# Go2Heart/StreamFormer

Hardware: AMD Instinct MI355X
Metric: frames/s (16x224^2 clips) (higher is better)
Workload: dtype bf16; 1 GPU; SigLIP-base StreamFormer encoder forward, 8 clips x 16 x 224^2 per GPU, random-init de-trivialised weights, causal temporal attention; global_batch_clips=8, frames_per_clip=16, parallelism=dp1, steps_in_flight=1

## Files before the change

include/streamformer_hip.h:

```cpp
#ifndef STREAMFORMER_HIP_H
#define STREAMFORMER_HIP_H

#include <stddef.h>
#include <stdint.h>

#ifdef __cplusplus
extern "C" {
#endif

typedef struct sf_encoder sf_encoder;
typedef struct sf_cache sf_cache;
typedef void* sf_stream;

typedef enum {
  SF_OK = 0,
  SF_ERR_INVALID = -1,
  SF_ERR_STATE = -2,
  SF_ERR_HIP = -3,
  SF_ERR_WORKSPACE = -4,
  SF_ERR_UNKNOWN_KEY = -5,
  SF_ERR_CAPACITY = -6
} sf_status;

typedef enum { SF_F32 = 0, SF_BF16 = 1, SF_F16 = 2, SF_F64 = 3, SF_U8 = 4 } sf_dtype;
// ... 395 lines not shown
int sf_op_crit_losses_backward(const float* const* pred_masks, int L, int B, int Q, int H, int W, const float* const* tgt_masks,
                               const int32_t* tgt_G, const int32_t* tgt_H, const int32_t* tgt_W, const int32_t* pairs_dev, int N,
                               const float* coords_dev, const float* sums_dev, int K, float num_masks, const float* upstream_dev,
                               float* grad_pred_masks_dev, sf_stream stream);
size_t sf_op_crit_class_loss_workspace_bytes(int L, int B, int Q);
int sf_op_crit_class_loss(const float* const* pred_logits, int L, int B, int Q, int C1, const int32_t* pairs_dev, int N,
                          const int64_t* const* tgt_labels, const int32_t* tgt_G, const float* weight_dev, float* losses_dev,
                          int losses_stride, float* grad_dev, int32_t* target_classes_out_dev, void* workspace, size_t workspace_bytes,
                          sf_stream stream);

int sf_op_clp_tracks(const float* embeds_dev, int R, int C, const int32_t* track_rows_dev, int T, int F, float* sg_dev, float* stats_dev,
                     sf_stream stream);
int sf_op_clp_items(const float* embeds_dev, int R, int C, const float* sg_dev, int T, int F, const int32_t* items_dev, int I,
                    const int32_t* neg_dev, int NE, int max_neg, float* losses_dev, float* item_out_dev, sf_stream stream);
size_t sf_op_clp_backward_workspace_bytes(int I, int T, int F, int C);
int sf_op_clp_backward(const float* embeds_dev, int R, int C, const float* sg_dev, const float* stats_dev, const int32_t* track_rows_dev,
                       const int32_t* track_items_dev, int T, int F, const int32_t* items_dev, int I, const int32_t* neg_dev, int NE,
                       int max_neg, const int32_t* row_start_dev, const int32_t* row_items_dev, const float* item_out_dev,
                       const float* upstream_dev, float* grad_embeds_dev, void* workspace, size_t workspace_bytes, sf_stream stream);

int sf_bench_gemm(sf_encoder* enc, int M, int which, int iters, void* workspace_dev,
                  size_t workspace_bytes, sf_stream stream, float* mean_ms_out, double* flops_out);

int sf_bench_attention(sf_encoder* enc, int B, int T, int which, int iters, void* workspace_dev,
                       size_t workspace_bytes, sf_stream stream, float* mean_ms_out, double* bytes_out,
                       double* flops_out);

void sf_reload_switches(void);
const char* sf_switch_info(int index, int what);

int sf_bench_launch_floor(int device, int launches, int iters, sf_stream stream, float* us_per_launch_out);

#ifdef __cplusplus
}
#endif
#endif
```

streamformer_amd/_native.py:

```python
from __future__ import annotations

import ctypes as C
import inspect
import os
import weakref

import torch

_HERE = os.path.dirname(os.path.abspath(__file__))
LIB_PATH = os.path.join(_HERE, "libstreamformer_hip.so")
if os.environ.get("SF_LIB"):
    LIB_PATH = os.path.join(_HERE, "libstreamformer_hip_%s.so" % os.environ["SF_LIB"])

SF_OK = 0
SF_ERR_INVALID, SF_ERR_STATE, SF_ERR_HIP, SF_ERR_WORKSPACE, SF_ERR_UNKNOWN_KEY, SF_ERR_CAPACITY = -1, -2, -3, -4, -5, -6
SF_F32, SF_BF16, SF_F16, SF_F64, SF_U8 = 0, 1, 2, 3, 4
SF_COMPUTE_BF16, SF_COMPUTE_BF16X3 = 0, 1


class SfConfig(C.Structure):
    _fields_ = [(n, C.c_int32) for n in (
        "image_size", "patch_size", "num_channels", "num_frames", "hidden_size", "num_hidden_layers",
        "num_attention_heads", "intermediate_size", "hidden_act", "qkv_bias", "enable_causal_temporal",
        "add_lora_spatial")] + [("layer_norm_eps", C.c_float)]
# ... 215 lines not shown
    "sf_op_seg_semantic": (_I, [_P, _P, _I, _I, _I, _I, _I, _I, _I, _I, _I, _I, _P, _P]),
    "sf_op_seg_panoptic_argmax": (_I, [_P, _P, _P, _I, _I, _F, _I, _I, _I, _I, _I, _I, _I, _I, _P, _P, _P]),
    "sf_op_seg_panoptic_relabel": (_I, [_P, _P, _I, C.c_longlong, _P, _P]),
    "sf_op_crit_costs_workspace_bytes": (_SZ, [_I, _I, _I, _I, _I]),
    "sf_op_crit_costs": (_I, [C.POINTER(_P), C.POINTER(_P), _I, _I, _I, _I, _I, _I, C.POINTER(_P), C.POINTER(_P), C.POINTER(C.c_int32),
                              C.POINTER(C.c_int32), C.POINTER(C.c_int32), _P, _I, _I, _F, _F, _F, _P, _P, _SZ, _P]),
    "sf_op_crit_losses_capacity": (_I, []),
    "sf_op_crit_losses_workspace_bytes": (_SZ, [_I]),
    "sf_op_crit_losses": (_I, [C.POINTER(_P), _I, _I, _I, _I, _I, C.POINTER(_P), C.POINTER(C.c_int32), C.POINTER(C.c_int32),
                               C.POINTER(C.c_int32), _P, C.POINTER(C.c_int32), _I, _P, _P, _I, _I, _I, _F, _P, _I, _P, _P, _P, _P, _SZ, _P]),
    "sf_op_crit_losses_backward": (_I, [C.POINTER(_P), _I, _I, _I, _I, _I, C.POINTER(_P), C.POINTER(C.c_int32), C.POINTER(C.c_int32),
                                        C.POINTER(C.c_int32), _P, _I, _P, _P, _I, _F, _P, _P, _P]),
    "sf_op_crit_class_loss_workspace_bytes": (_SZ, [_I, _I, _I]),
    "sf_op_crit_class_loss": (_I, [C.POINTER(_P), _I, _I, _I, _I, _P, _I, C.POINTER(_P), C.POINTER(C.c_int32), _P, _P, _I, _P, _P, _P, _SZ,
                                   _P]),
    "sf_op_clp_tracks": (_I, [_P, _I, _I, _P, _I, _I, _P, _P, _P]),
    "sf_op_clp_items": (_I, [_P, _I, _I, _P, _I, _I, _P, _I, _P, _I, _I, _P, _P, _P]),
    "sf_op_clp_backward_workspace_bytes": (_SZ, [_I, _I, _I, _I]),
    "sf_op_clp_backward": (_I, [_P, _I, _I, _P, _P, _P, _P, _I, _I, _P, _I, _P, _I, _I, _P, _P, _P, _P, _P, _P, _SZ, _P]),
    "sf_reload_switches": (None, []),
    "sf_switch_info": (C.c_char_p, [_I, _I]),
    "sf_bench_launch_floor": (_I, [_I, _I, _I, _P, C.POINTER(_F)]),
    "sf_bench_gemm": (_I, [_P, _I, _I, _I, _P, _SZ, _P, C.POINTER(_F), C.POINTER(C.c_double)]),
    "sf_bench_attention": (_I, [_P, _I, _I, _I, _I, _P, _SZ, _P, C.POINTER(_F), C.POINTER(C.c_double),
                                C.POINTER(C.c_double)]),
}


def _load() -> C.CDLL:
    if not os.path.exists(LIB_PATH):
        raise ImportError(
            f"{LIB_PATH} is missing: build it with `python streamformer_amd/build.py` "
            "(hipcc --offload-arch=gfx950).  There is no non-HIP fallback.")
    lib = C.CDLL(LIB_PATH, mode=C.RTLD_GLOBAL)
    for name, (res, args) in SIGNATURES.items():
        try:
            fn = getattr(lib, name)
        except AttributeError as e:
            raise ImportError(f"{LIB_PATH} does not export {name} (stale build? run "
                              "`python streamformer_amd/build.py`)") from e
        fn.restype = res
        fn.argtypes = args
    return lib


lib = _load()
# ... 165 lines not shown
```

streamformer_amd/csrc/sf_bench.hip:

```cpp
#include "sf_encoder.h"

#include <cstring>

template <typename Launch>
static hipError_t sf_time_launches(hipStream_t s, int iters, Launch&& launch, float* mean_ms) {
  hipEvent_t e0 = nullptr, e1 = nullptr;
  hipError_t err = hipEventCreate(&e0);
  if (err == hipSuccess) err = hipEventCreate(&e1);
  if (err == hipSuccess) err = launch();
  if (err == hipSuccess) err = hipEventRecord(e0, s);
  for (int i = 0; i < iters && err == hipSuccess; ++i) err = launch();
  if (err == hipSuccess) err = hipEventRecord(e1, s);
  if (err == hipSuccess) err = hipEventSynchronize(e1);
  float ms = 0.f;
  if (err == hipSuccess) err = hipEventElapsedTime(&ms, e0, e1);
  if (e0) (void)hipEventDestroy(e0);
  if (e1) (void)hipEventDestroy(e1);
  if (err == hipSuccess) *mean_ms = ms / iters;
  return err;
}

extern "C" int sf_bench_gemm(sf_encoder* e, int M, int which, int iters, void* workspace, size_t workspace_bytes,
                             sf_stream stream, float* mean_ms_out, double* flops_out) {
  if (!e || !e->finalized || e->layers.empty()) return sf_set_err(SF_ERR_STATE, "encoder not finalized");
  if (iters <= 0 || M <= 0 || !workspace || !mean_ms_out) return sf_set_err(SF_ERR_INVALID, "bad argument");
  const DevLayer& l = e->layers[0];
  const bool plain = which == 4 || which == 5;
  if (plain) which = which == 4 ? 3 : 1;
  const DevLinear* lin = which == 0 ? &l.up : which == 1 ? &l.down : which == 2 ? &l.s_qkv : &l.s_out;
  const bool acc = e->compute == SF_COMPUTE_BF16X3;
  const int epi = plain ? (acc ? SF_EPI_F32 : SF_EPI_BF16) : which == 0 ? SF_EPI_ACT_BF16 : which == 2 ? (acc ? SF_EPI_F32 : SF_EPI_BF16) : SF_EPI_RESID_F32;
  const bool pm = epi == SF_EPI_RESID_F32 && resid_planes_at(e, M);
  SfCarver c(workspace, acc || pm, true);
  const SfPlanes ap = c.planes((size_t)M * lin->K);
  SfPlanes op = c.planes((size_t)M * lin->N);
  float* of = c.take<float>((size_t)M * lin->N);
  if (c.off > workspace_bytes) return sf_set_err(SF_ERR_WORKSPACE, "workspace %zu < required %zu", workspace_bytes, c.off);
  hipStream_t s = (hipStream_t)stream;
  if (acc && epi == SF_EPI_RESID_F32) op.hi = nullptr;
  float* st = pm ? c.take<float>((size_t)M * 8) : nullptr;
  if (c.off > workspace_bytes) return sf_set_err(SF_ERR_WORKSPACE, "workspace %zu < required %zu", workspace_bytes, c.off);
  if (st) HIP_TRY(hipMemsetAsync(st, 0, (size_t)M * 8 * sizeof(float), (hipStream_t)stream));
  SfGemmArgs g = linear_args(e, *lin, ap.hi, ap.lo, M, epi, acc);
  g.alpha = 0.f; g.out_hi = op.hi; g.out_lo = op.lo;
  if (pm) { g.resid_hi = op.hi; g.resid_lo = op.lo; g.ln_stats_out = st; }
  else { g.out_f32 = of; g.resid = of; }
  HIP_TRY(sf_time_launches(s, iters, [&]() { return sf_launch_gemm(g, acc, s); }, mean_ms_out));
  if (flops_out) *flops_out = 2.0 * M * (double)lin->N * (double)lin->K;
  return SF_OK;
}

extern "C" int sf_bench_attention(sf_encoder* e, int B, int T, int which, int iters, void* workspace,
                                  size_t workspace_bytes, sf_stream stream, float* mean_ms_out, double* bytes_out,
                                  double* flops_out) {
  if (!e || !e->finalized) return sf_set_err(SF_ERR_STATE, "encoder not finalized");
  if (iters <= 0 || B <= 0 || T <= 0 || !workspace || !mean_ms_out) return sf_set_err(SF_ERR_INVALID, "bad argument");
  const bool acc = e->compute == SF_COMPUTE_BF16X3;
  const int D = e->D, N = e->N, heads = e->cfg.num_attention_heads;
  const size_t M = (size_t)B * T * N, esz = acc ? 4 : 2;
  SfCarver c(workspace);
  char* qkv = c.take<char>(M * 3 * D * esz);
  bf16_t* ch = c.take<bf16_t>(M * D);
  bf16_t* cl = c.take<bf16_t>(M * D);
  if (c.off > workspace_bytes) return sf_set_err(SF_ERR_WORKSPACE, "workspace %zu < required %zu", workspace_bytes, c.off);
  hipStream_t s = (hipStream_t)stream;
  HIP_TRY(hipMemsetAsync(qkv, 0x3c, M * 3 * D * esz, s));
  SfAttnArgs a;
  memset(&a, 0, sizeof(a));
  a.q = qkv; a.k = qkv + (size_t)D * esz; a.v = qkv + (size_t)2 * D * esz;
  a.in_is_f32 = acc; a.row_pitch_q = 3 * D; a.row_pitch_kv = 3 * D; a.heads = heads; a.scale = 0.125f;
  a.ctx_hi = ch; a.ctx_lo = cl; a.D = D; a.N = N;
  if (which == 0 && acc && sf_spatial_planes_ok(N, false)) {
// ... 66 lines not shown
```

streamformer_amd/csrc/sf_common.h:

```cpp
#pragma once
#include <hip/hip_runtime.h>
#include <stdint.h>

typedef unsigned short bf16_t;

typedef __attribute__((ext_vector_type(8))) short bf16x8_t;
typedef __attribute__((ext_vector_type(4))) float f32x4_t;
typedef __attribute__((ext_vector_type(4))) unsigned int u32x4_t;
typedef __attribute__((ext_vector_type(2))) unsigned int u32x2_t;

#define SF_DEVICE __device__ __forceinline__

#ifdef SF_LAB
#define SF_LAB_SWITCH(name) (getenv(name) ? atoi(getenv(name)) : 0)
#else
#define SF_LAB_SWITCH(name) 0
#endif

SF_DEVICE int sf_swz64(int row) {
#ifdef SF_SWZ64_LEGACY
  return (row >> 2) & 3;
#else
  return (0 - (row >> 2)) & 3;
#endif
// ... 200 lines not shown
  if (p.grp_rows <= 0) return (size_t)m;
  if (p.grp_tab) {
    const int g = m / p.grp_rows;
    const SfStreamSlot e = p.grp_tab[g];
    return (size_t)e.stream * p.grp_stride + e.slot * p.grp_off_scale + (m - g * p.grp_rows);
  }
  const int off = p.grp_off + (p.grp_off_dev ? *p.grp_off_dev * p.grp_off_scale : 0);
  return (size_t)(m / p.grp_rows) * p.grp_stride + off + (m % p.grp_rows);
}
int sf_wall_clock_ticks(int ns);
enum SfGemmFamily {
  SF_GEMM_FAM_NONE = 0,
  SF_GEMM_FAM_SKINNY = 1, SF_GEMM_FAM_TILE = 2, SF_GEMM_FAM_PANEL = 3, SF_GEMM_FAM_G256 = 4, SF_GEMM_FAM_G128 = 5,
  SF_GEMM_FAM_COLSPLIT = 6,
  SF_GEMM_FAM_LAB_PIPE = 7, SF_GEMM_FAM_LAB_PP = 8,
};
SfGemmFamily sf_gemm_family(const SfGemmArgs& a, bool split);
hipError_t sf_launch_gemm_family(SfGemmFamily fam, const SfGemmArgs& a, bool split, hipStream_t s);
hipError_t sf_launch_gemm(const SfGemmArgs& a, bool split, hipStream_t s);
bool sf_gemm128_supported(const SfGemmArgs& a, bool split);
hipError_t sf_launch_gemm128(const SfGemmArgs& a, bool split, hipStream_t s);
bool sf_gemm256_supported(const SfGemmArgs& a, bool split);
bool sf_gemm256_aux_supported(const SfGemmArgs& a);
hipError_t sf_launch_gemm256(const SfGemmArgs& a, hipStream_t s);
int sf_skinny_max_rows();
bool sf_gemm_skinny_supported(const SfGemmArgs& a, bool split);
hipError_t sf_launch_gemm_skinny(const SfGemmArgs& a, bool split, hipStream_t s);
bool sf_gemm_tile_supported(const SfGemmArgs& a, bool split);
hipError_t sf_launch_gemm_tile(const SfGemmArgs& a, hipStream_t s);
int sf_tile_max_rows();
int sf_tile_fold_min_rows();
int sf_infold_max_rows();
struct SfQkvArgs {
  const bf16_t* a;
  const bf16_t* w;
  const float* bias; const float* ln_s;
  const float* ln_stats; float ln_eps;
  int M, K, D;
  int B, T, NP;
  bf16_t* out;
  float scale; int causal;
};
bool sf_gemm_qkv_supported(const SfQkvArgs& a, bool fused);
hipError_t sf_launch_gemm_qkv(const SfQkvArgs& a, bool fused, hipStream_t s);
struct SfStreamQkvArgs {
  const bf16_t* a;
// ... 147 lines not shown
```

streamformer_amd/csrc/sf_encoder.h:

```cpp
#pragma once
#include "sf_handle.h"

#include <vector>

struct DevLinear : SfDevLinear {
  const float* ln_s = nullptr;
  const bf16_t* w_frag = nullptr;
};
using DevLN = SfDevLN;
struct DevLayer {
  DevLN ln_t, ln_b, ln_a;
  DevLinear t_qkv, t_out, t_dense, t_fused, s_qkv, s_out, up, down;
  DevLinear t_qkv_f, s_qkv_f, up_f;
  DevLinear t_qkv_fp;
  float gate_tanh = 0.f;
};

struct sf_encoder {
  sf_config cfg;
  int device = 0;
  int N = 0, D = 0, I = 0, L = 0, Kp = 0, hd = 64;
  SfWeightStore weights;
  bool finalized = false;
  int compute = SF_COMPUTE_BF16;
// ... 64 lines not shown
  int ready = 0;
  const SfStreamParams* sp = nullptr;
  const StreamPos* pos = nullptr;
  const SfStreamSlot* tab = nullptr;
};

enum EmbedRoute { EMBED_NONE, EMBED_TILE, EMBED_PANEL, EMBED_GEMM };

struct ForwardPlan {
  ForwardRequest rq;
  int N, M, F;
  bool acc;
  int qkv_epi; size_t esz;
  float scale;
  int t_row, slot, tk;
  bool zero_stats;
  bool time_folded;
  EmbedRoute embed_route;
  bf16_t* patches;
  SfGemmArgs embed;
  bool fold, sfold, xm, gm, pm;
  bool anyfold;
  bool rplanes;
  bool seed_stats;
  bool seed_split;
  float* resid;
  bf16_t* fold_hi;
  bf16_t* plo; bf16_t* plo2;
  float* fold_st;
  const bf16_t* ln_in; const bf16_t* ln_in_lo;
  bool tplanes, planes;
  size_t tsz, sesz;
  bool head_generic;
  bool head_rows;
};

struct FoldShape { bool tile_fold, small_fold, stats_fold; };

#pragma GCC visibility push(hidden)
int check_geometry(const sf_encoder* e, int B, int T, int H, int W, const float* pos_dev, int* N_out);
Workspace carve(const sf_encoder* e, void* base, int B, int T, int N, bool need_tqkv);
ForwardPlan plan_forward(const sf_encoder* e, const ForwardRequest& rq, const Workspace& ws);
int run_plan(sf_encoder* e, const ForwardPlan& p, const Workspace& ws, hipStream_t s);
int run_forward(sf_encoder* e, const ForwardRequest& rq, const Workspace& ws, hipStream_t s);
SfGemmArgs linear_args(const sf_encoder* e, const DevLinear& lin, const bf16_t* a_hi, const bf16_t* a_lo, int M, int epi, bool split);
bool resid_planes_at(const sf_encoder* e, int M, FoldShape* fs = nullptr);
#pragma GCC visibility pop
```

streamformer_amd/csrc/sf_encoder.hip:

```cpp
#include "sf_encoder.h"
#include "sf_switches.h"
#include "sf_pool_head.h"

#include <cmath>
#include <cstdarg>
#include <cstdio>
#include <cstdlib>
#include <cstring>
#include <string>
#include <vector>

#define SF_ABI_VERSION 5
static const int kLoraRank = 32;

static thread_local char g_err[1024] = "";
int sf_set_err(int code, const char* fmt, ...) {
  va_list ap;
  va_start(ap, fmt);
  vsnprintf(g_err, sizeof(g_err), fmt, ap);
  va_end(ap);
  return code;
}

static void build_expected(sf_encoder* e) {
// ... 431 lines not shown
static bool ln_fold_panel_ok(const sf_encoder* e, int M) {
  if (e->compute != SF_COMPUTE_BF16 || sf_sw(SW_DISABLE_LN_FOLD)) return false;
  return takes_both_k(e, probe_args(e, M, e->D, e->D, SF_EPI_RESID_F32), [](const SfGemmArgs& a) { return sf_gemm_panel_supported(a, false); }) &&
         bf16_consumers_on_g256(e, M);
}

static bool ln_fold_planes_g256_ok(const sf_encoder* e, int M, bool split) {
  if ((e->D % 256) || e->D > 1024) return false;
  SfGemmArgs g = probe_args(e, M, e->D, e->D, SF_EPI_RESID_F32);
  if (split) { g.a_lo = kSetB; g.w_lo = kSetB; }
  g.out_hi = kSetB; g.out_lo = kSetB; g.ln_stats_out = kSetF; g.resid_hi = kSetB; g.resid_lo = kSetB;
  if (!takes_both_k(e, g, [split](const SfGemmArgs& a) { return sf_gemm256_supported(a, split); })) return false;
  g.ln_stats_out = nullptr; g.resid_hi = g.resid_lo = nullptr; g.ln_stats = kSetF; g.ln_s = kSetF;
  if (split) g.out_hi = nullptr; else g.out_lo = nullptr;
  g.epi = SF_EPI_BF16; g.K = e->D; g.N = g.ldc = 3 * e->D;
  if (!sf_gemm256_supported(g, split)) return false;
  g.epi = SF_EPI_ACT_BF16; g.N = g.ldc = e->I;
  return sf_gemm256_supported(g, split);
}
static bool ln_fold_acc_ok(const sf_encoder* e, int M) {
  return e->compute == SF_COMPUTE_BF16X3 && !sf_sw(SW_DISABLE_ACC_FOLD) && ln_fold_planes_g256_ok(e, M, true);
}
static bool ln_fold_g256_ok(const sf_encoder* e, int M) {
  return e->compute == SF_COMPUTE_BF16 && !sf_sw(SW_DISABLE_LN_FOLD) && ln_fold_planes_g256_ok(e, M, false);
}

static bool ln_fold_small_ok(const sf_encoder* e, int M) {
  if (M > sf_infold_max_rows() || sf_sw(SW_DISABLE_STREAM_FOLD)) return false;
  const bool acc = e->compute == SF_COMPUTE_BF16X3;
  auto takes = [acc](const SfGemmArgs& g) { return sf_gemm_skinny_supported(g, acc) || (!acc && sf_gemm_tile_supported(g, false)); };
  SfGemmArgs g = probe_args(e, M, 3 * e->D, e->D, acc ? SF_EPI_F32 : SF_EPI_BF16);
  if (acc) { g.a_lo = kSetB; g.w_lo = kSetB; g.out_lo = kSetB; g.out_f32 = kSetF; }
  g.ln_inkernel = 1; g.ln_s = kSetF; g.out_hi = kSetB;
  if (!takes(g)) return false;
  g.epi = SF_EPI_ACT_BF16; g.N = g.ldc = e->I;
  if (!takes(g)) return false;
  g.ln_inkernel = 0; g.ln_s = nullptr; g.epi = SF_EPI_RESID_F32; g.N = g.ldc = e->D;
  g.out_f32 = kSetF; g.resid = kSetF;
  return takes_both_k(e, g, takes);
}

static bool sf_head_rows_ok(const sf_encoder* e, int F) {
  return e->head_out.w_lo && e->head_fc1.w_lo && e->head_fc2.w_lo && sf_rowlin_supported(F, e->D, e->D) && sf_rowlin_supported(F, e->I, e->D) &&
         sf_rowlin_supported(F, e->D, e->I);
}

static int time_rows(const sf_encoder* e, int t_past, int T, bool streaming, SfRowIndex* idx) {
// ... 1 lines not shown
  idx->n = T;
  if (streaming) {
    if (t_past + T > nf)
      return sf_set_err(SF_ERR_CAPACITY, "streaming needs time-embedding row %d but config.num_frames is %d", t_past + T - 1, nf);
    for (int t = 0; t < T; ++t) idx->idx[t] = t_past + t;
  } else if (T <= nf) {
    for (int t = 0; t < T; ++t) idx->idx[t] = t;
  } else {
    const float scale = (float)nf / (float)T;
    for (int t = 0; t < T; ++t) {
      int src = (int)floorf((float)t * scale);
      idx->idx[t] = src < nf - 1 ? src : nf - 1;
    }
  }
  return SF_OK;
}

bool resid_planes_at(const sf_encoder* e, int M, FoldShape* fs) {
  FoldShape f;
  f.tile_fold = ln_fold_tile_ok(e, M); f.small_fold = ln_fold_small_ok(e, M);
  f.stats_fold = f.tile_fold || (!f.small_fold && ln_fold_panel_ok(e, M));
  if (fs) *fs = f;
  return f.stats_fold && !f.tile_fold && e->compute != SF_COMPUTE_BF16X3 && !sf_sw(SW_DISABLE_RESID_PLANES);
}

ForwardPlan plan_forward(const sf_encoder* e, const ForwardRequest& rq, const Workspace& ws) {
  ForwardPlan p = {};
  p.rq = rq;
  if (p.rq.lb < 0) p.rq.lb = e->L;
  const int D = e->D, T = rq.T, stages = rq.stages;
  const int N = (rq.H / e->cfg.patch_size) * (rq.W / e->cfg.patch_size), M = rq.B * T * N;
  const bool acc = e->compute == SF_COMPUTE_BF16X3, streaming = rq.streaming;
  const bool complete = (stages & 7) == 7 && !rq.hidden_states;
  p.N = N; p.M = M; p.F = rq.B * T; p.acc = acc;
  p.qkv_epi = acc ? SF_EPI_F32 : SF_EPI_BF16; p.esz = acc ? 4 : 2;
  p.scale = 1.0f / sqrtf((float)e->hd);
  p.t_row = rq.pos ? rq.pos->t_row : rq.t_past; p.slot = rq.pos ? rq.pos->slot : rq.t_past; p.tk = rq.pos ? rq.pos->tk : rq.t_past + T;

  FoldShape fs;
  const bool resid_planes = resid_planes_at(e, M, &fs);
  const bool tile_fold = fs.tile_fold, small_fold = fs.small_fold, stats_fold = fs.stats_fold;
  const bool small_bufs = ws.res_bf && (!acc || ws.res_lo) && small_fold;
  p.zero_stats = stats_fold && !streaming && (stages & 3);

  const bool panel_embed = stats_fold && !streaming && (stages & 2) && ws.embed_tab && ws.patch_buf && e->Kp % 32 == 0 && e->Kp >= 128 && D == 768 &&
                           !sf_sw(SW_EMBED_VIA_GEMM128);
// ... 20 lines not shown
    SfGemmArgs gt = g;
    gt.out_hi = ws.xn_hi; gt.ln_stats_out = ws.ln_stats; gt.ln_stats_wide = 1;
    if (!acc && !streaming && (stages & 2) && p.patches != ws.xn_hi && tile_fold && sf_gemm_tile_supported(gt, false)) {
      p.embed_route = EMBED_TILE; p.embed = gt;
    } else if (panel_embed && sf_gemm_panel_supported(gp, false)) {
      p.embed_route = EMBED_PANEL; p.embed = gp;
    } else {
      p.time_folded = rq.sp && T == 1 && !stats_fold && !sf_sw(SW_DISABLE_SKINNY) && sf_gemm_skinny_supported(g, acc);
      if (p.time_folded) { g.time_rows = e->time_tab; g.time_base_dev = &rq.sp->t_row; g.grp_tab = rq.tab; }
      if (small_bufs && (stages & 2)) { g.out_hi = ws.res_bf; if (acc) g.out_lo = ws.res_lo; }
      p.embed_route = EMBED_GEMM; p.embed = g;
    }
  }

  p.tplanes = acc && !rq.layer_tqkv && rq.cap == T && rq.t_past == 0 && sf_temporal_planes_ok(T, T);
  p.planes = acc && sf_spatial_planes_ok(N, rq.attentions != nullptr);
  p.tsz = p.tplanes ? 2 : p.esz; p.sesz = p.planes ? 2 : p.esz;
  p.fold = stats_fold && !streaming;
  p.sfold = !p.fold && small_bufs;
  p.xm = p.tplanes && p.planes && !streaming && complete && ln_fold_acc_ok(e, M);
  p.gm = !acc && !p.fold && !p.sfold && !streaming && complete && ws.res_lo != nullptr && ln_fold_g256_ok(e, M);
  p.anyfold = p.fold || p.sfold || p.xm || p.gm;
  p.rplanes = p.pm || p.xm || p.gm;
  p.seed_stats = p.fold && (stages & 2) && p.embed_route != EMBED_TILE && p.embed_route != EMBED_PANEL;
  p.seed_split = p.sfold && (stages & 2) && !(stages & 1) && !(rq.ready & 2);
  p.resid = p.rplanes ? nullptr : ws.resid;
  p.fold_hi = (p.fold || p.xm || p.gm) ? ws.xn_hi : (p.sfold ? ws.res_bf : nullptr);
  p.fold_st = (p.fold || p.xm || p.gm) ? ws.ln_stats : nullptr;
  p.plo = (p.pm || p.gm) ? ws.res_lo : (p.xm ? ws.xn_lo : ((p.sfold && acc) ? ws.res_lo : nullptr));
  p.plo2 = (p.xm && !sf_sw(SW_ACC_TWO_PLANES)) ? ws.res_lo2 : nullptr;
  p.ln_in = p.sfold ? ws.res_bf : ws.xn_hi;
  p.ln_in_lo = (p.sfold && acc) ? ws.res_lo : ws.xn_lo;

  p.head_generic = e->hd != 64 || D > 1024;
  p.head_rows = rq.pooler && sf_head_rows_ok(e, p.F);
  return p;
}

static hipError_t launch_resid_linear(const sf_encoder* e, const ForwardPlan& p, const DevLinear& lin, const bf16_t* a_hi, const bf16_t* a_lo,
                                      float alpha, hipStream_t s) {
  SfGemmArgs g = linear_args(e, lin, a_hi, a_lo, p.M, SF_EPI_RESID_F32, p.acc);
  g.alpha = alpha;
  g.resid = p.resid; g.out_f32 = p.resid;
  g.resid_hi = p.rplanes ? p.fold_hi : nullptr; g.resid_lo = p.plo; g.resid_lo2 = p.plo2;
  g.out_hi = p.fold_hi; g.out_lo = p.plo; g.out_lo2 = p.plo2;
  g.ln_stats_out = p.fold_st;
  return sf_launch_gemm(g, p.acc, s);
}

static SfGemmArgs ln_linear_args(const sf_encoder* e, const ForwardPlan& p, const DevLinear& plain, const DevLinear& folded, int epi) {
  const DevLinear& lin = p.anyfold ? folded : plain;
  SfGemmArgs g = linear_args(e, lin, p.ln_in, p.ln_in_lo, p.M, epi, p.acc);
  g.ln_stats = p.fold_st; g.ln_inkernel = p.sfold;
  g.ln_s = (p.fold_st || p.sfold) ? lin.ln_s : nullptr;
  return g;
}
static void set_qkv_out(SfGemmArgs& g, void* qkv, bool planes, const ForwardPlan& p) {
  if (planes) g.epi = SF_EPI_BF16;
  g.out_f32 = (float*)qkv; g.out_hi = (bf16_t*)qkv;
  g.out_lo = planes ? (bf16_t*)qkv + (size_t)p.M * g.N : nullptr;
}
static void set_qkv_in(SfAttnArgs& a, const sf_encoder* e, void* qkv, bool planes, size_t esz, const ForwardPlan& p, const Workspace& ws) {
  const int D = e->D;
  a.q = qkv; a.k = (char*)qkv + (size_t)D * esz; a.v = (char*)qkv + (size_t)2 * D * esz;
  a.in_is_f32 = p.acc && !planes; a.lo_plane_off = planes ? (long long)p.M * 3 * D : 0;
  a.row_pitch_q = 3 * D; a.row_pitch_kv = 3 * D; a.heads = e->cfg.num_attention_heads; a.scale = p.scale; a.head_dim = e->hd;
  a.N = p.N; a.ctx_hi = ws.ctx_hi; a.ctx_lo = ws.ctx_lo; a.D = D;
}

// ... 332 lines not shown
```

streamformer_amd/csrc/sf_gemm256.hip:

```cpp
#include "sf_common.h"
#include "sf_switches.h"
#include <cstdlib>

#define G_THREADS 512
#define PIECE_BYTES 16384

typedef const __attribute__((address_space(1))) void* gptr_t;
typedef __attribute__((address_space(3))) void* lptr_t;

SF_DEVICE f32x4_t mfma16b(bf16x8_t a, bf16x8_t b, f32x4_t c) {
  typedef __attribute__((ext_vector_type(8))) __bf16 v8bf;
  return __builtin_amdgcn_mfma_f32_16x16x32_bf16(__builtin_bit_cast(v8bf, a), __builtin_bit_cast(v8bf, b), c, 0, 0, 0);
}

SF_DEVICE bf16x8_t rd_frag(const char* piece, int row, int kc) {
  return *reinterpret_cast<const bf16x8_t*>(piece + row * 128 + ((kc ^ ((row >> 1) & 7)) << 4));
}
SF_DEVICE bf16x8_t rd_frag_s(const char* piece, int plane, int row, int g) {
  return *reinterpret_cast<const bf16x8_t*>(piece + plane * 8192 + row * 64 + ((g ^ sf_swz64(row)) << 4));
}

#ifdef SF_G256_TRACE
__device__ unsigned long long g256_trace[16];
#endif
// ... 405 lines not shown
                const f32x4_t& vv = j < 2 ? v0 : v1;
                x[2 * j] = (bf2f(hi[j] & 0xffffu) + bf2f(li[j] & 0xffffu)) + bf2f(l2i[j] & 0xffffu) + p.alpha * vv[(2 * j) & 3];
                x[2 * j + 1] = (bf2f(hi[j] >> 16) + bf2f(li[j] >> 16)) + bf2f(l2i[j] >> 16) + p.alpha * vv[(2 * j + 1) & 3];
              }
              u32x4_t h, l, l2;
#pragma unroll
              for (int j = 0; j < 4; ++j) {
                h[j] = pack_bf2(x[2 * j], x[2 * j + 1]);
                const float r0 = x[2 * j] - bf2f(h[j] & 0xffffu), r1 = x[2 * j + 1] - bf2f(h[j] >> 16);
                l[j] = pack_bf2(r0, r1);
                l2[j] = pack_bf2(r0 - bf2f(l[j] & 0xffffu), r1 - bf2f(l[j] >> 16));
                s1 += x[2 * j] + x[2 * j + 1];
                s2 += x[2 * j] * x[2 * j] + x[2 * j + 1] * x[2 * j + 1];
              }
              *reinterpret_cast<u32x4_t*>(p.out_hi + o) = h;
              *reinterpret_cast<u32x4_t*>(p.out_lo + o) = l;
              if (p.out_lo2) *reinterpret_cast<u32x4_t*>(p.out_lo2 + o) = l2;
            }
#pragma unroll
            for (int sh = 1; sh <= 16; sh <<= 1) {
              s1 += __shfl_xor(s1, sh, 64);
              s2 += __shfl_xor(s2, sh, 64);
            }
            if (ok && c2 == 0)
              *reinterpret_cast<u32x2_t*>(p.ln_stats_out + (size_t)m * 8 + (size_t)(n0 >> 8) * 2) = (u32x2_t){__float_as_uint(s1), __float_as_uint(s2)};
          }
        } else {
#pragma unroll 4
          for (int it = 0; it < 16; ++it) {
            const int idx = it * G_THREADS + tid;
            const int r = idx >> 6, c = idx & 63;
            f32x4_t v = *reinterpret_cast<const f32x4_t*>(smem + r * 1024 + ((c ^ (r & 63)) << 4));
            const int m = m0 + (r >> 6) * HR + mq * 64 + (r & 63);
            if (m < p.M && (r & 63) < (mq ? MT1 : 4) * 16) {
              size_t orow = (size_t)m;
              if (p.grp_rows > 0) orow = sf_out_row(p, m);
              const size_t o = orow * (size_t)p.ldc + n0 + c * 4;
              if (EPI == SF_EPI_RESID_F32) v = *reinterpret_cast<const f32x4_t*>(p.resid + o) + p.alpha * v;
              *reinterpret_cast<f32x4_t*>(p.out_f32 + o) = v;
            }
          }
        }
        __syncthreads();
      }
    }
  }
}

bool sf_gemm256_supported(const SfGemmArgs& a, bool split) {
  if (split && (!a.a_lo || !a.w_lo || a.aux_mode || sf_sw(SW_DISABLE_G256_SPLIT))) return false;
  if (split && a.ln_stats && (!a.ln_stats_wide || !a.ln_s || (a.K % 256) || a.K > 1024 || (a.epi != SF_EPI_BF16 && a.epi != SF_EPI_ACT_BF16))) return false;
  if (a.epi == SF_EPI_EMBED_F32) return false;
  bool planes = false;
  if (a.epi == SF_EPI_RESID_F32 && a.out_hi) {
    if (!a.out_lo || !a.resid_hi || !a.resid_lo || !a.ln_stats_out || !a.ln_stats_wide || (a.N % 256) || a.N > 1024 || a.grp_rows > 0) return false;
    if (!split && (a.resid_lo2 || a.out_lo2)) return false;
    planes = true;
  } else if (a.resid_hi) {
    return false;
  }
  if (!split && a.epi == SF_EPI_ACT_BF16 && a.act != 0 && a.act != 99) return false;
  if (a.K % 128 || a.K < 128) return false;
  int min_n = 1024;
  if (split) {
    min_n = a.M <= 6272 ? 1024 : 768;
    if (const char* e = sf_sw(SW_G256_SPLIT_MIN_N)) min_n = atoi(e);
  }
  if (a.N % 256 || a.N < min_n) return false;
  if (a.M < 2048 || (size_t)a.M * a.K * 2 >= ((size_t)1 << 32) || (size_t)a.N * a.K * 2 >= ((size_t)1 << 32)) return false;
  if (a.out_lo && !split && !planes) return false;
  return true;
}

bool sf_gemm256_aux_supported(const SfGemmArgs& a) {
  return a.epi == SF_EPI_BF16 && a.aux != nullptr && sf_gemm256_supported(a, false);
}

static int g256_grid() {
  int cus = sf_device_cus();
  if (cus < 8) cus = 256;
  return cus & ~7;
}

template <int BM, bool SPLIT_ONLY = false>
static hipError_t launch_bm(const SfGemmArgs& a_in, hipStream_t s) {
  SfGemmArgs a = a_in;
  if (SF_LAB_SWITCH("SF_G256_LAB_NOSTORE")) a.act = 99;
  const int tiles = ((a.M + BM - 1) / BM) * (a.N / 256);
  const size_t lds = 8 * PIECE_BYTES;
  const dim3 grid(g256_grid()), block(G_THREADS);
  int stagger = 0, sgroups = 3;
  if (const char* ge = sf_sw(SW_G256_STAGGER_GROUPS)) sgroups = atoi(ge) > 1 ? atoi(ge) : 2;
  {
    const int rounds = (tiles + (int)grid.x - 1) / (int)grid.x;
    double pct = 21.0;
    if (const char* pe = sf_sw(SW_G256_STAGGER_PCT)) pct = atof(pe);
    const char* env = sf_sw(SW_G256_STAGGER_NS);
    if (env) stagger = sf_wall_clock_ticks(atoi(env));
    else if (rounds >= 3) {
      const double mfma_x = (a.a_lo && a.w_lo) ? 3.0 : 1.0;
      const double tile_ns = mfma_x * 2.0 * BM * 256.0 * a.K / 3.9e3 + 6500.0;
      stagger = sf_wall_clock_ticks((int)(tile_ns * pct / 100.0));
    }
  }
// ... 2 lines not shown
  }
  {
    int cg = 0;
    if (const char* we = sf_sw(SW_G256_WALK)) cg = atoi(we);
    if (cg < 0 || cg > 15 || (cg != 15 && cg >= a.N / 256)) cg = 0;
    sgroups = (sgroups & 255) | (cg << 8) | (sf_sw(SW_G256_STORE_WT) ? 1 << 12 : 0) | (sf_sw(SW_G256_STORE_NT) ? 1 << 13 : 0);
  }
#define SF_LAUNCH256(E, L, SP) return sf_launch_big_lds(sf_gemm256_kernel<E, L, BM, SP>, grid, block, lds, s, a, tiles, stagger, sgroups)
  if (a.a_lo && a.w_lo) {
    if (a.aux_mode) return hipErrorInvalidValue;
    if (a.ln_stats) {
      if (!a.ln_stats_wide || !a.ln_s) return hipErrorInvalidValue;
      if (a.epi == SF_EPI_BF16) SF_LAUNCH256(SF_EPI_BF16, true, true);
      if (a.epi == SF_EPI_ACT_BF16) SF_LAUNCH256(SF_EPI_ACT_BF16, true, true);
      return hipErrorInvalidValue;
    }
    switch (a.epi) {
#define SF_CASE(E) case E: SF_LAUNCH256(E, false, true);
      SF_CASE(SF_EPI_F32) SF_CASE(SF_EPI_BF16) SF_CASE(SF_EPI_ACT_BF16) SF_CASE(SF_EPI_RESID_F32)
#undef SF_CASE
      default: return hipErrorInvalidValue;
    }
  }
  if constexpr (SPLIT_ONLY) return hipErrorInvalidValue;
  else {
  const bool lnf = a.ln_stats != nullptr;
  if (lnf && (!a.ln_s || (a.epi != SF_EPI_BF16 && a.epi != SF_EPI_ACT_BF16))) return hipErrorInvalidValue;
  switch (a.epi) {
    case SF_EPI_F32: SF_LAUNCH256(SF_EPI_F32, false, false);
    case SF_EPI_BF16:
      if (a.aux_mode) {
        if (lnf || !a.aux) return hipErrorInvalidValue;
        SF_LAUNCH256(G256_EPI_BF16_AUX, false, false);
      }
      if (lnf) SF_LAUNCH256(SF_EPI_BF16, true, false);
      SF_LAUNCH256(SF_EPI_BF16, false, false);
    case SF_EPI_ACT_BF16:
      if (lnf) SF_LAUNCH256(SF_EPI_ACT_BF16, true, false);
      SF_LAUNCH256(SF_EPI_ACT_BF16, false, false);
    case SF_EPI_RESID_F32: SF_LAUNCH256(SF_EPI_RESID_F32, false, false);
    default: return hipErrorInvalidValue;
  }
  }
#undef SF_LAUNCH256
}

hipError_t sf_launch_gemm256(const SfGemmArgs& a, hipStream_t s) {
  const int g = g256_grid(), nt = a.N / 256;
  auto cost = [&](int bm) { const int tiles = ((a.M + bm - 1) / bm) * nt; return (long)((tiles + g - 1) / g) * bm; };
  if (a.a_lo && a.w_lo && !sf_sw(SW_G256_NO_SHORT_BM)) {
    auto t = [&](int bm, double f) { return (double)cost(bm) / bm * f; };
    const double t256 = t(256, 1632), t224 = t(224, 1472), t192 = t(192, 1370), t160 = t(160, 1268);
    const double best = fmin(fmin(t256, t224), fmin(t192, t160));
    if (const char* fe = sf_sw(SW_G256_FORCE_BM)) {
      switch (atoi(fe)) { case 160: return launch_bm<160, true>(a, s); case 192: return launch_bm<192, true>(a, s); case 224: return launch_bm<224>(a, s); default: return launch_bm<256>(a, s); }
    }
    if (best == t160 && t160 < 0.97 * fmin(t224, t256)) return launch_bm<160, true>(a, s);
    if (best == t192 && t192 < 0.97 * fmin(t224, t256)) return launch_bm<192, true>(a, s);
  }
  if (cost(224) < cost(256) && !sf_sw(SW_G256_NO_BM224)) return launch_bm<224>(a, s);
  return launch_bm<256>(a, s);
}
```

streamformer_amd/csrc/sf_gemm_panel.hip:

```cpp
#include "sf_common.h"
#include "sf_switches.h"
#include <cstdlib>

#define P_THREADS 512
#define P_NT 3
#define P_SLOT_BYTES 40960
#define P_A_BYTES 16384

typedef __attribute__((address_space(3))) void* lptr_t;

SF_DEVICE f32x4_t mfma16p(bf16x8_t a, bf16x8_t b, f32x4_t c) {
  typedef __attribute__((ext_vector_type(8))) __bf16 v8bf;
  return __builtin_amdgcn_mfma_f32_16x16x32_bf16(__builtin_bit_cast(v8bf, a), __builtin_bit_cast(v8bf, b), c, 0, 0, 0);
}
template <int N>
SF_DEVICE void wait_vmp() {
  asm volatile("s_waitcnt vmcnt(%0)" ::"n"(N) : "memory");
}
SF_DEVICE bf16x8_t rd32(const char* piece, int row, int kc) {
  return *reinterpret_cast<const bf16x8_t*>(piece + row * 64 + ((kc ^ sf_swz64(row)) << 4));
}

#ifdef SF_PANEL_TRACE
__device__ unsigned long long panel_trace[16];
// ... 224 lines not shown
              *reinterpret_cast<u32x2_t*>(p.out_hi + o) = hv;
              if (p.out_lo)
                *reinterpret_cast<u32x2_t*>(p.out_lo + o) = (u32x2_t){pack_bf2(x[0] - bf2f(hv[0] & 0xffffu), x[1] - bf2f(hv[0] >> 16)),
                                                                    pack_bf2(x[2] - bf2f(hv[1] & 0xffffu), x[3] - bf2f(hv[1] >> 16))};
              s1 += (x[0] + x[1]) + (x[2] + x[3]);
              s2 += (x[0] * x[0] + x[1] * x[1]) + (x[2] * x[2] + x[3] * x[3]);
            }
          }
        }
        if (p.ln_stats_out) {
          s1 = wave_sum_dpp(s1);
          s2 = wave_sum_dpp(s2);
          if (elane == 0) {
            p.ln_stats_out[(size_t)m * 8 + nh * 4 + 0] = s1;
            p.ln_stats_out[(size_t)m * 8 + nh * 4 + 1] = s2;
          }
        }
      }
    }
    PT_MARK(3);
    __syncthreads();
    PT_MARK(4);
  }
  PT_FLUSH();
  }
}

static int panel_cus() {
  int cus = sf_device_cus();
  if (cus < 16) cus = 256;
  return cus & ~15;
}

struct PanelPlan { int panels, rows, mt, ok; };
static PanelPlan panel_plan(int M) {
  PanelPlan pl = {0, 0, 0, 0};
  const int half = panel_cus() / 2;
  int panels = ((M + 207) / 208 + half - 1) / half * half;
  if (panels <= 0) return pl;
  const int rows = (M + panels - 1) / panels;
  static const int kMt[4] = {2, 4, 7, 13};
  for (int i = 0; i < 4; ++i)
    if (rows <= 16 * kMt[i]) { pl.mt = kMt[i]; break; }
  if (!pl.mt) return pl;
  const int forced = sf_sw(SW_PANEL_MIN_FILL_PCT) ? atoi(sf_sw(SW_PANEL_MIN_FILL_PCT)) : 0;
  const int min_fill = forced ? forced : (M >= 14000 ? 55 : 75);
// ... 38 lines not shown
```

streamformer_amd/csrc/sf_switches.h:

```cpp
#pragma once

#define SF_SWITCH_TABLE(X) \
  X(ACC_TWO_PLANES, "SF_ACC_TWO_PLANES", "accurate mode: residual stream as two planes instead of three (A/B; max-abs 1.4e-4 instead of 5e-5)") \
  X(ASSUME_CUS, "SF_ASSUME_CUS", "size persistent grids for this many CUs (CU-masked stream experiments)") \
  X(DISABLE_ACC_FOLD, "SF_DISABLE_ACC_FOLD", "accurate mode: fp32 residual + standalone LayerNorm instead of the folded plane form (A/B)") \
  X(DISABLE_G256_SPLIT, "SF_DISABLE_G256_SPLIT", "accurate mode: keep the bf16x3 GEMMs off the persistent 256-column kernel") \
  X(DISABLE_GEMM_COLSPLIT, "SF_DISABLE_GEMM_COLSPLIT", "N = 256 j + 128 (so400m widths): the whole GEMM on 128^2 tiles instead of 256-column kernel + a 128-column tail (A/B)") \
  X(DISABLE_GEMM_MID, "SF_DISABLE_GEMM_MID", "skinny family: no 64 x 64 tiles above 512 rows") \
  X(DISABLE_GEMM_TILE, "SF_DISABLE_GEMM_TILE", "one / two clips per call: no tile-GEMM family") \
  X(DISABLE_LN_FOLD, "SF_DISABLE_LN_FOLD", "bf16 mode: standalone LayerNorm launches instead of the fold into the consumer GEMMs (A/B)") \
  X(DISABLE_RESID_PLANES, "SF_DISABLE_RESID_PLANES", "bf16 mode: fp32 residual stream instead of hi + lo planes (A/B)") \
  X(DISABLE_SKG_UNROLL, "SF_DISABLE_SKG_UNROLL", "streaming: K-parallel skinny GEMM with a run-time K-tile count (A/B)") \
  X(DISABLE_SKINNY, "SF_DISABLE_SKINNY", "send small-M GEMMs to the generic 128^2 kernel") \
  X(DISABLE_SPATIAL_DMA, "SF_DISABLE_SPATIAL_DMA", "spatial attention on the register-staged kernel") \
  X(DISABLE_SPATIAL_DMA_ACC, "SF_DISABLE_SPATIAL_DMA_ACC", "accurate mode: spatial attention on fp32 q / k / v (test coverage of that path)") \
  X(DISABLE_SPATIAL_NTC, "SF_DISABLE_SPATIAL_NTC", "spatial attention with a run-time tile count (A/B)") \
  X(DISABLE_STREAM_FOLD, "SF_DISABLE_STREAM_FOLD", "streaming: standalone LayerNorm launches (A/B)") \
  X(DISABLE_STREAM_GRAPH, "SF_DISABLE_STREAM_GRAPH", "streaming: eager launches instead of hipGraph replay") \
  X(DISABLE_TEMPORAL_DECODE, "SF_DISABLE_TEMPORAL_DECODE", "streaming: general temporal kernel instead of the single-query one") \
  X(TBWD_OWN_CU, "SF_TBWD_OWN_CU", "training: temporal attention backward as 12-wave workgroups that own a CU instead of 4-wave workgroups with their exact LDS (bit-identical, 65 against 51 us per launch; for jobs that share a device, DESIGN.md 4)") \
  X(TEMPORAL_DECODE_LANE_KEY, "SF_TEMPORAL_DECODE_LANE_KEY", "streaming: single-query temporal kernel with one key per lane (A/B against whole-line loads)") \
  X(DISABLE_TEMPORAL_DMA, "SF_DISABLE_TEMPORAL_DMA", "temporal attention on the register-staged kernel") \
  X(DISABLE_TEMPORAL_DMA_ACC, "SF_DISABLE_TEMPORAL_DMA_ACC", "accurate mode: temporal attention on fp32 q / k / v (test coverage of that path)") \
  X(EMBED_VIA_GEMM128, "SF_EMBED_VIA_GEMM128", "embedding GEMM on the generic kernel (A/B)") \
  X(G256_FORCE_BM, "SF_G256_FORCE_BM", "256-column kernel: force the row-tile height (tests of the short tiles)") \
  X(G256_NO_BM224, "SF_G256_NO_BM224", "256-column kernel: no 224-row tiles") \
  X(G256_NO_SHORT_BM, "SF_G256_NO_SHORT_BM", "256-column kernel, accurate mode: no 160 / 192-row tiles") \
  X(G256_SPLIT_MIN_N, "SF_G256_SPLIT_MIN_N", "accurate mode: smallest N the persistent kernel takes") \
  X(G256_WALK, "SF_G256_WALK", "256-column kernel: column-group width (tiles) of the column-group-major tile walk, 0 = row-major (A/B of the fabric traffic)") \
  X(G256_STORE_WT, "SF_G256_STORE_WT", "256-column kernel: bf16 outputs leave with write-through (sc1) stores that do not stay in the XCD's L2 (A/B)") \
  X(G256_STORE_NT, "SF_G256_STORE_NT", "256-column kernel: bf16 outputs leave with non-temporal stores (A/B: do the residual planes then survive in the Infinity Cache?)") \
  X(G256_STAGGER_GROUPS, "SF_G256_STAGGER_GROUPS", "256-column kernel: phase-stagger groups per XCD") \
  X(G256_STAGGER_NS, "SF_G256_STAGGER_NS", "256-column kernel: stagger step in ns (overrides the percentage)") \
  X(G256_STAGGER_ONLY, "SF_G256_STAGGER_ONLY", "256-column kernel: stagger only some launches (A/B)") \
  X(G256_STAGGER_PCT, "SF_G256_STAGGER_PCT", "256-column kernel: stagger step as a percentage of the tile period") \
  X(GEMM_MID_MIN_M, "SF_GEMM_MID_MIN_M", "skinny family: first M of the 64 x 64 tiles") \
  X(LN_BWD_BLOCKS, "SF_LN_BWD_BLOCKS", "LayerNorm backward: workgroups (tuning)") \
  X(POOL_SHARE_CU, "SF_POOL_SHARE_CU", "pooling head: the probe / combine kernels request only the LDS they use instead of a CU's whole 160 KB (A/B; with it other workgroups share their CUs, see DESIGN.md 4 on device sharing)") \
  X(PANEL_MIN_FILL_PCT, "SF_PANEL_MIN_FILL_PCT", "panel kernel: minimum last-round fill") \
  X(PANEL_PAD_CLAMP, "SF_PANEL_PAD_CLAMP", "panel kernel: clamp instead of zero-fill the padding rows (A/B)") \
  X(PANEL_STAGGER_NS, "SF_PANEL_STAGGER_NS", "panel kernel: phase-stagger step in ns") \
  X(SKINNY_MAX_M, "SF_SKINNY_MAX_M", "skinny family: largest M") \
  X(SKINNY_NO_KG, "SF_SKINNY_NO_KG", "skinny family: no K-parallel variant") \
  X(SKINNY_NB, "SF_SKINNY_NB", "streaming, folded skinny consumers: 1 = 32 x 32 tiles everywhere, 2 / 3 = force 32 x 64 / 32 x 96 tiles (A/B)") \
  X(SKINNY_NT, "SF_SKINNY_NT", "skinny family: non-temporal weight loads (A/B)") \
  X(SKINNY_TPS, "SF_SKINNY_TPS", "skinny family: tiles per slot (tuning)") \
  X(SPATIAL_PERS, "SF_SPATIAL_PERS", "lab library: persistent spatial attention kernel") \
  X(SPATIAL_TPW, "SF_SPATIAL_TPW", "spatial attention: query tiles per workgroup (tuning)") \
  X(STREAM_GRAPH_PER_POSITION, "SF_STREAM_GRAPH_PER_POSITION", "streaming: one graph per cache position instead of the position-free one (A/B)") \
  X(TILE_FOLD_MIN_M, "SF_TILE_FOLD_MIN_M", "tile-GEMM family: smallest M whose LayerNorm fold uses a statistics buffer and the 256^2 consumers") \
  X(TILE_MAX_M, "SF_TILE_MAX_M", "tile-GEMM family: largest M") \
  X(TILE_MIN_M, "SF_TILE_MIN_M", "tile-GEMM family: smallest M") \
  X(TILE_SHAPE, "SF_TILE_SHAPE", "tile-GEMM family: force a tile shape (tools/tile_lab.py)") \
  X(TRAIN_UNFUSED_TEMPORAL, "SF_TRAIN_UNFUSED_TEMPORAL", "training: temporal_attention.output.dense and temporal_dense as two launches instead of one fused projection (A/B)") \
  X(TRAIN_SIDE_STREAM, "SF_TRAIN_SIDE_STREAM", "training: 0 keeps the LoRA gradients on the caller stream (A/B)") \
  X(WGRAD_NSPLIT, "SF_WGRAD_NSPLIT", "weight-gradient GEMM: force the token splits") \
  X(WGRAD_SMALL_TILES, "SF_WGRAD_SMALL_TILES", "weight-gradient GEMM: 128^2 tiles only") \
  X(WGRAD_UNGROUPED, "SF_WGRAD_UNGROUPED", "training: one weight-gradient launch per projection instead of one per layer (test / A/B)") \

enum SfSw {
#define SF_SW_ENUM(id, name, what) SW_##id,
  SF_SWITCH_TABLE(SF_SW_ENUM)
#undef SF_SW_ENUM
  SW_COUNT
// ... 3 lines not shown
```

Before: 15580 frames/s.

## Route K=768 residual projections to 256-column plane producer with 160-row tiles

Adds a path that sends the bf16 residual-epilogue projections with K = D = 768 (N = 768) to the 256-column GEMM kernel, using 160-row tiles over two rounds instead of the panel kernel's single lock-step round. Both kernels now zero the unused LayerNorm statistics slots so the downstream fold reads consistent stats. The 256-column LayerNorm fold is disabled for D = 768. The goal is better CU fill and tile efficiency for these projections, at the cost of a second round and a different producer.

```diff
diff --git a/include/streamformer_hip.h b/include/streamformer_hip.h
--- a/include/streamformer_hip.h
+++ b/include/streamformer_hip.h
@@ -441,6 +441,8 @@
 int sf_bench_gemm(sf_encoder* enc, int M, int which, int iters, void* workspace_dev,
                   size_t workspace_bytes, sf_stream stream, float* mean_ms_out, double* flops_out);
 
+int sf_resid_family(sf_encoder* enc, int M, int K);
+
 int sf_bench_attention(sf_encoder* enc, int B, int T, int which, int iters, void* workspace_dev,
                        size_t workspace_bytes, sf_stream stream, float* mean_ms_out, double* bytes_out,
                        double* flops_out);
diff --git a/streamformer_amd/_native.py b/streamformer_amd/_native.py
--- a/streamformer_amd/_native.py
+++ b/streamformer_amd/_native.py
@@ -261,6 +261,7 @@
     "sf_switch_info": (C.c_char_p, [_I, _I]),
     "sf_bench_launch_floor": (_I, [_I, _I, _I, _P, C.POINTER(_F)]),
     "sf_bench_gemm": (_I, [_P, _I, _I, _I, _P, _SZ, _P, C.POINTER(_F), C.POINTER(C.c_double)]),
+    "sf_resid_family": (_I, [_P, _I, _I]),
     "sf_bench_attention": (_I, [_P, _I, _I, _I, _I, _P, _SZ, _P, C.POINTER(_F), C.POINTER(C.c_double),
                                 C.POINTER(C.c_double)]),
 }
diff --git a/streamformer_amd/csrc/sf_bench.hip b/streamformer_amd/csrc/sf_bench.hip
--- a/streamformer_amd/csrc/sf_bench.hip
+++ b/streamformer_amd/csrc/sf_bench.hip
@@ -45,9 +45,15 @@
   g.alpha = 0.f; g.out_hi = op.hi; g.out_lo = op.lo;
   if (pm) { g.resid_hi = op.hi; g.resid_lo = op.lo; g.ln_stats_out = st; }
   else { g.out_f32 = of; g.resid = of; }
-  HIP_TRY(sf_time_launches(s, iters, [&]() { return sf_launch_gemm(g, acc, s); }, mean_ms_out));
+  const SfGemmFamily fam = (pm && resid_on_g256_at(e, M, lin->K)) ? SF_GEMM_FAM_G256 : sf_gemm_family(g, acc);
+  HIP_TRY(sf_time_launches(s, iters, [&]() { return sf_launch_gemm_family(fam, g, acc, s); }, mean_ms_out));
   if (flops_out) *flops_out = 2.0 * M * (double)lin->N * (double)lin->K;
   return SF_OK;
+}
+
+extern "C" int sf_resid_family(sf_encoder* e, int M, int K) {
+  if (!e || !e->finalized || M <= 0 || (K != e->D && K != e->I) || !resid_planes_at(e, M)) return SF_GEMM_FAM_NONE;
+  return resid_on_g256_at(e, M, K) ? SF_GEMM_FAM_G256 : SF_GEMM_FAM_PANEL;
 }
 
 extern "C" int sf_bench_attention(sf_encoder* e, int B, int T, int which, int iters, void* workspace,
diff --git a/streamformer_amd/csrc/sf_common.h b/streamformer_amd/csrc/sf_common.h
--- a/streamformer_amd/csrc/sf_common.h
+++ b/streamformer_amd/csrc/sf_common.h
@@ -246,6 +246,7 @@
 hipError_t sf_launch_gemm128(const SfGemmArgs& a, bool split, hipStream_t s);
 bool sf_gemm256_supported(const SfGemmArgs& a, bool split);
 bool sf_gemm256_aux_supported(const SfGemmArgs& a);
+bool sf_gemm256_resid_rounds_ok(const SfGemmArgs& a);
 hipError_t sf_launch_gemm256(const SfGemmArgs& a, hipStream_t s);
 int sf_skinny_max_rows();
 bool sf_gemm_skinny_supported(const SfGemmArgs& a, bool split);
diff --git a/streamformer_amd/csrc/sf_encoder.h b/streamformer_amd/csrc/sf_encoder.h
--- a/streamformer_amd/csrc/sf_encoder.h
+++ b/streamformer_amd/csrc/sf_encoder.h
@@ -110,6 +110,7 @@
   bool fold, sfold, xm, gm, pm;
   bool anyfold;
   bool rplanes;
+  bool r256;
   bool seed_stats;
   bool seed_split;
   float* resid;
@@ -133,4 +134,5 @@
 int run_forward(sf_encoder* e, const ForwardRequest& rq, const Workspace& ws, hipStream_t s);
 SfGemmArgs linear_args(const sf_encoder* e, const DevLinear& lin, const bf16_t* a_hi, const bf16_t* a_lo, int M, int epi, bool split);
 bool resid_planes_at(const sf_encoder* e, int M, FoldShape* fs = nullptr);
+bool resid_on_g256_at(const sf_encoder* e, int M, int K);
 #pragma GCC visibility pop
diff --git a/streamformer_amd/csrc/sf_encoder.hip b/streamformer_amd/csrc/sf_encoder.hip
--- a/streamformer_amd/csrc/sf_encoder.hip
+++ b/streamformer_amd/csrc/sf_encoder.hip
@@ -477,7 +477,7 @@
   return e->compute == SF_COMPUTE_BF16X3 && !sf_sw(SW_DISABLE_ACC_FOLD) && ln_fold_planes_g256_ok(e, M, true);
 }
 static bool ln_fold_g256_ok(const sf_encoder* e, int M) {
-  return e->compute == SF_COMPUTE_BF16 && !sf_sw(SW_DISABLE_LN_FOLD) && ln_fold_planes_g256_ok(e, M, false);
+  return e->compute == SF_COMPUTE_BF16 && !sf_sw(SW_DISABLE_LN_FOLD) && e->D != 768 && ln_fold_planes_g256_ok(e, M, false);
 }
 
 static bool ln_fold_small_ok(const sf_encoder* e, int M) {
@@ -525,6 +525,14 @@
   f.stats_fold = f.tile_fold || (!f.small_fold && ln_fold_panel_ok(e, M));
   if (fs) *fs = f;
   return f.stats_fold && !f.tile_fold && e->compute != SF_COMPUTE_BF16X3 && !sf_sw(SW_DISABLE_RESID_PLANES);
+}
+
+bool resid_on_g256_at(const sf_encoder* e, int M, int K) {
+  const char* sw = sf_sw(SW_RESID_G256);
+  if ((sw && !atoi(sw)) || K != e->D) return false;
+  SfGemmArgs g = probe_args(e, M, e->D, K, SF_EPI_RESID_F32);
+  g.out_hi = kSetB; g.out_lo = kSetB; g.ln_stats_out = kSetF; g.resid_hi = kSetB; g.resid_lo = kSetB;
+  return sf_gemm256_supported(g, false) && sf_gemm256_resid_rounds_ok(g);
 }
 
 ForwardPlan plan_forward(const sf_encoder* e, const ForwardRequest& rq, const Workspace& ws) {
@@ -591,6 +599,7 @@
   p.gm = !acc && !p.fold && !p.sfold && !streaming && complete && ws.res_lo != nullptr && ln_fold_g256_ok(e, M);
   p.anyfold = p.fold || p.sfold || p.xm || p.gm;
   p.rplanes = p.pm || p.xm || p.gm;
+  p.r256 = p.fold && p.pm && resid_on_g256_at(e, M, D);
   p.seed_stats = p.fold && (stages & 2) && p.embed_route != EMBED_TILE && p.embed_route != EMBED_PANEL;
   p.seed_split = p.sfold && (stages & 2) && !(stages & 1) && !(rq.ready & 2);
   p.resid = p.rplanes ? nullptr : ws.resid;
@@ -614,6 +623,7 @@
   g.resid_hi = p.rplanes ? p.fold_hi : nullptr; g.resid_lo = p.plo; g.resid_lo2 = p.plo2;
   g.out_hi = p.fold_hi; g.out_lo = p.plo; g.out_lo2 = p.plo2;
   g.ln_stats_out = p.fold_st;
+  if (p.r256 && g.K == e->D) return sf_launch_gemm_family(SF_GEMM_FAM_G256, g, p.acc, s);
   return sf_launch_gemm(g, p.acc, s);
 }
 
diff --git a/streamformer_amd/csrc/sf_gemm256.hip b/streamformer_amd/csrc/sf_gemm256.hip
--- a/streamformer_amd/csrc/sf_gemm256.hip
+++ b/streamformer_amd/csrc/sf_gemm256.hip
@@ -451,8 +451,11 @@
               s1 += __shfl_xor(s1, sh, 64);
               s2 += __shfl_xor(s2, sh, 64);
             }
-            if (ok && c2 == 0)
+            if (ok && c2 == 0) {
               *reinterpret_cast<u32x2_t*>(p.ln_stats_out + (size_t)m * 8 + (size_t)(n0 >> 8) * 2) = (u32x2_t){__float_as_uint(s1), __float_as_uint(s2)};
+              if (n0 + 256 == p.N)
+                for (int q = tiles_n; q < 4; ++q) *reinterpret_cast<u32x2_t*>(p.ln_stats_out + (size_t)m * 8 + (size_t)q * 2) = (u32x2_t){0u, 0u};
+            }
           }
         } else {
 #pragma unroll 4
@@ -490,13 +493,15 @@
   }
   if (!split && a.epi == SF_EPI_ACT_BF16 && a.act != 0 && a.act != 99) return false;
   if (a.K % 128 || a.K < 128) return false;
-  int min_n = 1024;
-  if (split) {
+  int min_n = 1024, min_m = 2048;
+  if (planes && !split) {
+    min_n = 768; min_m = 1;
+  } else if (split) {
     min_n = a.M <= 6272 ? 1024 : 768;
     if (const char* e = sf_sw(SW_G256_SPLIT_MIN_N)) min_n = atoi(e);
   }
   if (a.N % 256 || a.N < min_n) return false;
-  if (a.M < 2048 || (size_t)a.M * a.K * 2 >= ((size_t)1 << 32) || (size_t)a.N * a.K * 2 >= ((size_t)1 << 32)) return false;
+  if (a.M < min_m || (size_t)a.M * a.K * 2 >= ((size_t)1 << 32) || (size_t)a.N * a.K * 2 >= ((size_t)1 << 32)) return false;
   if (a.out_lo && !split && !planes) return false;
   return true;
 }
@@ -509,6 +514,14 @@
   int cus = sf_device_cus();
   if (cus < 8) cus = 256;
   return cus & ~7;
+}
+
+static bool g256_planes768(const SfGemmArgs& a) { return a.epi == SF_EPI_RESID_F32 && a.resid_hi && !(a.a_lo && a.w_lo) && a.N == 768; }
+static constexpr int kPlanes768Bm = 160;
+bool sf_gemm256_resid_rounds_ok(const SfGemmArgs& a) {
+  if (!g256_planes768(a)) return false;
+  const int g = g256_grid(), tiles = ((a.M + kPlanes768Bm - 1) / kPlanes768Bm) * 3, rounds = (tiles + g - 1) / g;
+  return rounds >= 2 && (tiles - (rounds - 1) * g) * 100 >= g * 80;
 }
 
 template <int BM, bool SPLIT_ONLY = false>
@@ -557,8 +570,10 @@
       default: return hipErrorInvalidValue;
     }
   }
-  if constexpr (SPLIT_ONLY) return hipErrorInvalidValue;
-  else {
+  if constexpr (SPLIT_ONLY) {
+    if (a.epi == SF_EPI_RESID_F32 && a.resid_hi) SF_LAUNCH256(SF_EPI_RESID_F32, false, false);
+    return hipErrorInvalidValue;
+  } else {
   const bool lnf = a.ln_stats != nullptr;
   if (lnf && (!a.ln_s || (a.epi != SF_EPI_BF16 && a.epi != SF_EPI_ACT_BF16))) return hipErrorInvalidValue;
   switch (a.epi) {
@@ -583,6 +598,7 @@
 hipError_t sf_launch_gemm256(const SfGemmArgs& a, hipStream_t s) {
   const int g = g256_grid(), nt = a.N / 256;
   auto cost = [&](int bm) { const int tiles = ((a.M + bm - 1) / bm) * nt; return (long)((tiles + g - 1) / g) * bm; };
+  if (g256_planes768(a)) return launch_bm<kPlanes768Bm, true>(a, s);
   if (a.a_lo && a.w_lo && !sf_sw(SW_G256_NO_SHORT_BM)) {
     auto t = [&](int bm, double f) { return (double)cost(bm) / bm * f; };
     const double t256 = t(256, 1632), t224 = t(224, 1472), t192 = t(192, 1370), t160 = t(160, 1268);
diff --git a/streamformer_amd/csrc/sf_gemm_panel.hip b/streamformer_amd/csrc/sf_gemm_panel.hip
--- a/streamformer_amd/csrc/sf_gemm_panel.hip
+++ b/streamformer_amd/csrc/sf_gemm_panel.hip
@@ -270,6 +270,8 @@
     __syncthreads();
     PT_MARK(4);
   }
+  if (p.ln_stats_out)
+    for (int m = m0 + tid_e; m < m_end; m += P_THREADS) *reinterpret_cast<u32x2_t*>(p.ln_stats_out + (size_t)m * 8 + nh * 4 + 2) = (u32x2_t){0u, 0u};
   PT_FLUSH();
   }
 }
diff --git a/streamformer_amd/csrc/sf_switches.h b/streamformer_amd/csrc/sf_switches.h
--- a/streamformer_amd/csrc/sf_switches.h
+++ b/streamformer_amd/csrc/sf_switches.h
@@ -40,6 +40,7 @@
   X(PANEL_MIN_FILL_PCT, "SF_PANEL_MIN_FILL_PCT", "panel kernel: minimum last-round fill") \
   X(PANEL_PAD_CLAMP, "SF_PANEL_PAD_CLAMP", "panel kernel: clamp instead of zero-fill the padding rows (A/B)") \
   X(PANEL_STAGGER_NS, "SF_PANEL_STAGGER_NS", "panel kernel: phase-stagger step in ns") \
+  X(RESID_G256, "SF_RESID_G256", "bf16 mode, eight clips per call and up: 0 = the K = 768 residual projections on the panel kernel (one lock-step round) instead of the 256^2 plane producer (two rounds of 160-row tiles) (A/B)") \
   X(SKINNY_MAX_M, "SF_SKINNY_MAX_M", "skinny family: largest M") \
   X(SKINNY_NO_KG, "SF_SKINNY_NO_KG", "skinny family: no K-parallel variant") \
   X(SKINNY_NB, "SF_SKINNY_NB", "streaming, folded skinny consumers: 1 = 32 x 32 tiles everywhere, 2 / 3 = force 32 x 64 / 32 x 96 tiles (A/B)") \
```

New measurement: 15650 frames/s (median of 3 runs). No clear change (+0.5%).
